# AlexGeControl/Visual-Inertial-Odometry

Measured on AMD Instinct MI355X. Metric: GN iterations/s, 11-frame (10-keyframe) window, 20k landmarks per GPU, higher is better.
Workload: dtype f64

## Files before the change

### visual-inertial-odometry_amd/csrc/vio_chain_core.h

```cpp
#ifndef VIO_CHAIN_CORE_H
#define VIO_CHAIN_CORE_H
#ifndef CH_DIAG_SKIP
#define CH_DIAG_SKIP 0
#endif

#ifdef VIO_STAMPS
#define CH_STAMP(slot) do { if (dbg && (tid & 63) == 0) { asm volatile("s_waitcnt lgkmcnt(0)" ::: "memory"); dbg[slot] = __builtin_amdgcn_s_memtime() - t_start__; } } while (0)
#else
#define CH_STAMP(slot) do { } while (0)
#endif

#ifdef VIO_STAMPS
__device__ unsigned long long *g_ch_dbg = nullptr;
__device__ unsigned long long g_ch_t0 = 0;
#define CH_TSTAMP(cond, slot) do { if ((cond) && g_ch_dbg && (threadIdx.x & 63) == 0) { g_ch_dbg[slot] = __builtin_amdgcn_s_memtime() - g_ch_t0; } } while (0)
#else
#define CH_TSTAMP(cond, slot) do { } while (0)
#endif
struct ChLane {
    int oA0, oA2;
    int oM0, oM2;
    int r16, g;
    bool r9;
};

__device__ __forceinline__ void ch_scan_tiles(double *P, int wi, int lane) {
    int *sNZ = (int *)(P + CH_OFF_NZ);
    for (int tile = wi; tile < 55; tile += 14) {
        const double *t = P + CH_OFF_SC + tile * CH_SCSZ;
        bool nz = t[lane] != 0.0 || t[lane + 64] != 0.0;
        if (lane + 128 < CH_SCSZ) nz = nz || t[lane + 128] != 0.0;
        const unsigned long long any = __ballot(nz);
        if (lane == 0) sNZ[tile] = any != 0ull ? 1 : 0;
    }
}
__device__ __forceinline__ unsigned long long ch_eff_mask(const double *P, int lane) {
    const int *sNZ = (const int *)(P + CH_OFF_NZ);
    const unsigned long long nz = __ballot(lane < 55 && sNZ[min(lane, 54)] != 0);
    unsigned long long eff = 0ull;
    unsigned a = 0, b = 0;
    for (int e = 0; e < 5; ++e) {
        a |= (unsigned)(nz >> (5 * e)) & 31u;
        b |= (unsigned)(nz >> (5 * (10 - e))) & 31u;
        eff |= (unsigned long long)a << (5 * e);
        eff |= (unsigned long long)b << (5 * (10 - e));
    }
    eff |= (unsigned long long)(((unsigned)(nz >> 25) & 31u) | a | b) << 25;
    return eff;
}
__device__ __forceinline__ bool ch_bit(unsigned long long eff, int e, int t) { return (eff >> (5 * e + t)) & 1ull; }

__device__ __forceinline__ void ch_chain_level(double *P, const ChLane &L, int e, int n, bool upd, int lane, double *scr) {
    double *sD = P + CH_OFF_D;
#ifdef VIO_STAMPS
    const unsigned long long ts0 = __builtin_amdgcn_s_memtime();
#endif
    if (e == 5) ch_factor<9, CH_TS, CH_TS>((lds_double *)(P + ch_sd(e)), (lds_double *)(P + CH_OFF_I9), (lds_double *)(P + ch_sm(e)), lane);
    else ch_factor<9, CH_TS, CH_TS, true>((lds_double *)(P + ch_sd(e)), (lds_double *)(P + CH_OFF_I9), (lds_double *)(P + ch_sm(e)), lane,
                                          (lds_double *)(P + ch_so(e)), (lds_double *)scr);
#ifdef VIO_STAMPS
    const unsigned long long ts1 = __builtin_amdgcn_s_memtime();
#endif
// ... 238 lines not shown
                ps_v4d acc2;
                ch_ld_c9(P + ch_sc(eB - 1, 0) + (wi - 5) * CH_SCSZ, L, acc2);
                ch_fused<eB, true>(P, L, wi - 5, acc2);
                ch_st_c9(P + ch_sc(eB - 1, 0) + (wi - 5) * CH_SCSZ, L, acc2);
            }
        }
        first_cc = wi >= 10 ? wi - 10 : wi + 3;
    } else {
        busy = wi < 5;
        if (wi < 5) {
            if (LEV == 4) {
                if (ch_bit(eff, 4, wi) || ch_bit(eff, 6, wi)) {
                    ps_v4d acc2;
                    ch_ld_c9(P + ch_sc(5, 0) + wi * CH_SCSZ, L, acc2);
                    if (ch_bit(eff, 4, wi)) ch_fused<4, true>(P, L, wi, acc2);
                    if (ch_bit(eff, 6, wi)) ch_fused<6, true>(P, L, wi, acc2);
                    ch_st_c9(P + ch_sc(5, 0) + wi * CH_SCSZ, L, acc2);
                }
            } else if (ch_bit(eff, 5, wi)) {
                ps_v4d dummy = {0.0, 0.0, 0.0, 0.0};
                ch_fused<5, false>(P, L, wi, dummy);
            }
        }
        first_cc = wi >= 5 ? wi - 5 : wi + 8;
    }
    if (CAM && LEV > 0 && wi < 5) {
        if (ch_bit(eff, LEV - 1, wi)) ch_yc_tile(P, LEV - 1, wi, lane);
        if (ch_bit(eff, 11 - LEV, wi)) ch_yc_tile(P, 11 - LEV, wi, lane);
    }
    if (CAM && LEV > 0) {
        if (LEV < 4) {
            if (wi >= 10 && wi < 13) { ch_cc_early(P, L, 2 * (wi - 10), LEV - 1, eff); ch_cc_early(P, L, 2 * (wi - 10) + 1, LEV - 1, eff); }
            else if (wi < 9) ch_cc_early(P, L, 6 + wi, LEV - 1, eff);
        } else if (wi < 5) {
            ch_cc_early(P, L, 10 + wi, LEV - 1, eff);
        } else if (wi < 13) {
            ch_cc_early(P, L, wi - 5, LEV - 1, eff);
            if (wi < 7) ch_cc_early(P, L, wi + 3, LEV - 1, eff);
        }
    }
    (void)first_cc;
    (void)busy;
}

__device__ __forceinline__ ChLane ch_lane(int lane) {
    const int r16 = lane & 15, g = lane >> 4;
    ChLane L;
    L.r16 = r16; L.g = g; L.r9 = r16 < 9;
    L.oA0 = r16 * CH_TS + g; L.oA2 = r16 * CH_TS + (g == 0 ? 8 : 9);
    L.oM0 = g * CH_TS + r16; L.oM2 = (g == 0) ? 8 * CH_TS + r16 : 8 * CH_TS + 9;
    return L;
}

template <bool CAM>
__device__ __forceinline__ unsigned long long ch_chain_elimination(double *P, const int tid, const ChLane &L, unsigned long long *dbg, unsigned long long t_start__,
                                                                   const bool scanned = false) {
    const int lane = tid & 63;
    const int uwave = __builtin_amdgcn_readfirstlane(tid >> 6);
    const int g = L.g;
    const bool r9 = L.r9;
    double *sD = P + CH_OFF_D;
    (void)dbg; (void)t_start__;
    unsigned long long eff = 0ull;
#ifndef CH_NO_PRIO
    if (uwave < 2) __builtin_amdgcn_s_setprio(3);
    else if (uwave == 15) __builtin_amdgcn_s_setprio(2);
#endif
    if (uwave < 2) {
        const int dir = uwave == 0 ? 1 : -1;
        int e = uwave == 0 ? 0 : 10;
        for (int lev = 0; lev < 6; ++lev, e += dir) {
            if (lev < 5 || uwave == 0) {
                if (lev == 5) {
                    double *td = P + ch_sd(5);
                    const double *so = P + ch_so(6);
                    const double a0 = so[L.oA0], a1 = so[L.oA0 + 4], a2 = so[L.oA2];
                    const double p0 = sD[6 * 16 + g], p1 = sD[6 * 16 + g + 4], p2 = sD[6 * 16 + g + 8];
                    ps_v4d acc = {td[L.oM0], td[L.oM0 + 4 * CH_TS], td[L.oM0 + 8 * CH_TS], 0.0};
                    acc = __builtin_amdgcn_mfma_f64_16x16x4f64(a0 * p0, -a0, acc, 0, 0, 0);
                    acc = __builtin_amdgcn_mfma_f64_16x16x4f64(a1 * p1, -a1, acc, 0, 0, 0);
                    acc = __builtin_amdgcn_mfma_f64_16x16x4f64(a2 * p2, -a2, acc, 0, 0, 0);
                    if (r9) { td[L.oM0] = acc[0]; td[L.oM0 + 4 * CH_TS] = acc[1]; if (g == 0) td[L.oM0 + 8 * CH_TS] = acc[2]; }
                }
                ch_chain_level(P, L, e, e + dir, !(uwave == 1 && lev == 4), lane, P + CH_OFF_X + 64 * uwave);
                if (uwave == 0) CH_STAMP(64 + 4 * lev);
            }
            CH_STAMP(256 + 16 * lev + uwave);
            __syncthreads();
            if (uwave == 0) CH_STAMP(65 + 4 * lev);
        }
        eff = ch_eff_mask(P, lane);
        if (uwave == 0) CH_STAMP(233);
        if (CAM) {
            if (uwave == 0) { if (ch_bit(eff, 5, 0)) { ps_v4d dummy = {0.0, 0.0, 0.0, 0.0}; ch_fused<5, false>(P, L, 0, dummy); } }
            else ch_cc_early(P, L, 0, 4, eff);
            if (uwave == 0) CH_STAMP(234);
            if (uwave == 1) CH_STAMP(235);
        }
        __syncthreads();
    } else {
        const int wi = uwave - 2;
        if (!scanned) ch_scan_tiles(P, wi, lane);
        CH_STAMP(256 + uwave);
        __syncthreads();
        eff = ch_eff_mask(P, lane);
        ch_worker_phase<0, CAM>(P, L, wi, lane, eff); if (uwave == 2) CH_STAMP(112);
        CH_STAMP(256 + 16 + uwave);
        __syncthreads();
        ch_worker_phase<1, CAM>(P, L, wi, lane, eff); if (uwave == 2) CH_STAMP(113);
        CH_STAMP(256 + 32 + uwave);
        __syncthreads();
        ch_worker_phase<2, CAM>(P, L, wi, lane, eff); if (uwave == 2) CH_STAMP(114); CH_STAMP(140 + uwave);
        CH_STAMP(256 + 48 + uwave);
        __syncthreads();
        ch_worker_phase<3, CAM>(P, L, wi, lane, eff); if (uwave == 2) CH_STAMP(115);
        CH_STAMP(256 + 64 + uwave);
        __syncthreads();
        ch_worker_phase<4, CAM>(P, L, wi, lane, eff); if (uwave == 2) CH_STAMP(116); CH_STAMP(180 + uwave);
        CH_STAMP(256 + 80 + uwave);
        __syncthreads();
        if (CAM) {
            if (wi >= 1 && wi < 5) { if (ch_bit(eff, 5, wi)) { ps_v4d dummy = {0.0, 0.0, 0.0, 0.0}; ch_fused<5, false>(P, L, wi, dummy); } }
            else if (wi == 13) ch_rhs_phase<5>(P, lane);
            else if (wi == 0 || (wi >= 5 && wi < 9)) {
                const int t = wi == 0 ? 0 : wi - 4;
                if (ch_bit(eff, 4, t)) ch_yc_tile(P, 4, t, lane);
                if (ch_bit(eff, 6, t)) ch_yc_tile(P, 6, t, lane);
            }
        } else {
            ch_worker_phase<5, CAM>(P, L, wi, lane, eff);
        }
        if (uwave == 2) CH_STAMP(117); CH_STAMP(200 + uwave);
        __syncthreads();
    }
    if (uwave == 0) CH_STAMP(87);
    return eff;
}

template <bool SPLIT, typename Mid1, typename Mid2>
__device__ __forceinline__ void ch_camera_solve(double *P, const int tid, const ChLane &L, const unsigned long long eff, Mid1 mid1, Mid2 mid2,
                                                unsigned long long *dbg, unsigned long long t_start__, const bool ext_trivial = false) {
    const int lane = tid & 63;
    const int uwave = __builtin_amdgcn_readfirstlane(tid >> 6);
    const int r16 = L.r16, g = L.g;
    const bool r9 = L.r9;
    double *sD = P + CH_OFF_D, *sX = P + CH_OFF_X, *sY = P + CH_OFF_Y, *sMc = P + CH_OFF_MC;
    (void)dbg; (void)t_start__;
    const int lofs = r16 * PS_TROW + g;
    const int cofs = g * PS_TROW + r16;
    if (SPLIT) {
#ifndef CH_NO_PRIO
        if (uwave == 0) __builtin_amdgcn_s_setprio(3);
        else if (uwave == 15) __builtin_amdgcn_s_setprio(2);
#endif
        if (uwave < 15) {
            int I, J;
            ch_tile_ij(uwave, I, J);
            double *tc = P + ch_cc(I, J) + cofs;
            ps_v4d acc;
#pragma unroll
            for (int v = 0; v < 4; ++v) acc[v] = tc[4 * PS_TROW * v];
            ch_cc_deferred_terms(P, L, I, J, acc, eff);
#pragma unroll
            for (int v = 0; v < 4; ++v) tc[4 * PS_TROW * v] = acc[v];
            if (uwave == 0) ch_factor_tile(P + ch_cc(0, 0), sMc, sD + CH_YC, 16, lane);
            else if (uwave >= 10) {
                const int t = uwave - 10;
#pragma unroll
                for (int i = 0; i < 11; ++i) {
                    const int e = (i == 10) ? 5 : ((i & 1) ? 10 - (i >> 1) : (i >> 1));
                    if (ch_bit(eff, e, t)) ch_yc_tile(P, e, t, lane);
                }
            }
        }
    } else
    if (uwave == 0) {
        double *tc = P + ch_cc(0, 0) + cofs;
        ps_v4d acc;
#pragma unroll
        for (int v = 0; v < 4; ++v) acc[v] = tc[4 * PS_TROW * v];
        if (ch_bit(eff, 5, 0)) ch_cc_term(P, L, 5, 0, 0, acc);
#pragma unroll
        for (int v = 0; v < 4; ++v) tc[4 * PS_TROW * v] = acc[v];
        ch_factor_tile(P + ch_cc(0, 0), sMc, sD + CH_YC, 16, lane);
    } else if (uwave == 15) {
        ch_yc_term<5>(P, lane);
    } else {
#ifndef CH_PREAMBLE_ALL_WAVES
        if ((uwave & 3) != 0) {
            ch_cc_last3(P, L, uwave, eff);
            if (uwave <= 3) ch_cc_last3(P, L, 4 * uwave, eff);
        }
#else
// ... 135 lines not shown
                if (g == 3) sX[CH_YC + 64 + r16] = x;
                __builtin_amdgcn_wave_barrier();
                asm volatile("" ::: "memory");
            }
            {
                const double *src = P + ch_cc(K, K) + r16 * PS_TROW;
#pragma unroll
                for (int j = 0; j < 16; ++j) mw[j] = src[j];
            }
#pragma unroll
            for (int J = 4; J >= 1; --J) {
                const double *src = P + ch_cc(J, min(K, J - 1)) + r16;
#pragma unroll
                for (int r = 0; r < 16; ++r) ucol[r] = src[r * PS_TROW];
                const double xj = sX[CH_YC + 16 * J + r16];
                PS_DOT16(acc, acc, xj, ucol);
                if (J >= 1) {
                    double x;
                    PS_DOT16(x, 0.0, own_v - acc, mw);
                    if (K == J - 1) sX[CH_YC + 16 * K + r16] = x;
                    __builtin_amdgcn_wave_barrier();
                    asm volatile("" ::: "memory");
                }
            }
        } else if (uwave < 11 && uwave != 5 && CH_DIAG_SKIP != 4) {
            const int e = uwave;
            const double *m = P + ch_sm(e) + k9 * CH_TS, *so = P + ch_so(e);
            double gk[3], mv[9], sv[3][9];
#pragma unroll
            for (int i = 0; i < 9; ++i) mv[i] = m[i];
#pragma unroll
            for (int v = 0; v < 3; ++v) {
                const int j = min(g + 4 * v, 8);
#pragma unroll
                for (int i = 0; i < 9; ++i) sv[v][i] = so[j * CH_TS + i];
            }
            __builtin_amdgcn_sched_barrier(0);
#pragma unroll
            for (int v = 0; v < 3; ++v) {
                double sum = 0.0;
#pragma unroll
                for (int i = 0; i < 9; ++i) sum = fma(mv[i], sv[v][i], sum);
                gk[v] = sum;
            }
            __builtin_amdgcn_sched_barrier(0);
            if (r9) {
                double *sg = P + ch_so(e) + k9 * CH_TS;
                sg[g] = gk[0]; sg[g + 4] = gk[1];
                if (g == 0) sg[8] = gk[2];
            }
        }
        if (uwave == 0) CH_STAMP(111);
        if (uwave == 15) CH_STAMP(170);
        __syncthreads();
        if ((uwave == 11 || uwave == 12) && CH_DIAG_SKIP != 4) {
            double gc[5][9], vc[5];
#pragma unroll
            for (int s2 = 0; s2 < 5; ++s2) {
                const int eb = (uwave == 11) ? 4 - s2 : 6 + s2;
                const double *src = P + ch_so(eb) + k9 * CH_TS;
#pragma unroll
                for (int j = 0; j < 9; ++j) gc[s2][j] = src[j];
            }
            __syncthreads();
            if (lane < 16) {
                double xs = sX[5 * 16 + k9];
#pragma unroll
                for (int s2 = 0; s2 < 5; ++s2) vc[s2] = sX[((uwave == 11) ? 4 - s2 : 6 + s2) * 16 + k9];
#pragma unroll
                for (int s2 = 0; s2 < 5; ++s2) {
                    const int eb = (uwave == 11) ? 4 - s2 : 6 + s2;
                    double t;
                    CH_DOT9(t, 0.0, xs, gc[s2]);
                    const double xn = vc[s2] - t;
                    if (r9) sX[eb * 16 + r16] = xn;
                    xs = xn;
                }
            }
            if (uwave == 11) CH_STAMP(175);
        } else {
            if (uwave == 13) {
                mid1(lane);
                CH_STAMP(171);
            } else if (uwave < 11 && CH_DIAG_SKIP != 4) {
                const int e = uwave;
                double sacc = 0.0, lv[5][4], xv[5][4];
#pragma unroll
                for (int t = 0; t < 5; ++t) {
                    if (ch_bit(eff, e, t)) {
                        const double *src = P + ch_sc(e, t) + g * CH_TS + k9;
                        const double *xj = sX + CH_YC + 16 * t + g;
#pragma unroll
                        for (int v = 0; v < 4; ++v) { lv[t][v] = src[4 * v * CH_TS]; xv[t][v] = xj[4 * v]; }
                    }
                }
                __builtin_amdgcn_sched_barrier(0);
#pragma unroll
                for (int t = 0; t < 5; ++t) {
                    if (ch_bit(eff, e, t)) {
#pragma unroll
                        for (int v = 0; v < 4; ++v) sacc = fma(lv[t][v], xv[t][v], sacc);
                    }
                }
                double *scr = P + CH_OFF_SD;
                scr[e * 64 + lane] = sacc;
                __builtin_amdgcn_wave_barrier();
                if (lane < 16) {
                    const double c = ((scr[e * 64 + r16] + scr[e * 64 + 16 + r16]) + scr[e * 64 + 32 + r16]) + scr[e * 64 + 48 + r16];
                    const double dd = sD[e * 16 + k9];
                    const double v = d_div(sY[e * 16 + k9], dd, d_fast_rcp(dd)) - c;
                    const double *src = P + ch_sm(e) + k9 * CH_TS;
                    double m9[9], gv;
#pragma unroll
                    for (int j = 0; j < 9; ++j) m9[j] = (j < k9) ? 0.0 : src[j];
                    CH_DOT9(gv, 0.0, v, m9);
                    if (r9) sX[e * 16 + r16] = gv;
                }
            }
            if (uwave == 0) CH_STAMP(172);
            __syncthreads();
            if (uwave == 0) CH_STAMP(173);
            mid2(uwave < 11 ? uwave : uwave - 2, lane);
            if (uwave == 0) CH_STAMP(174);
        }
        if (uwave == 0) CH_STAMP(63);
        d_lds_barrier();
    }
}

template <typename Mid1, typename Mid2>
__device__ __forceinline__ void ch_factor_solve(double *P, const int tid, Mid1 mid1, Mid2 mid2, unsigned long long *dbg = nullptr, const bool ext_trivial = false,
                                                const bool scanned = false) {
    unsigned long long t_start__ = 0ull;
#ifdef VIO_STAMPS
    t_start__ = __builtin_amdgcn_s_memtime();
    if (tid == 0) { g_ch_dbg = dbg; g_ch_t0 = t_start__; }
#endif
    const ChLane L = ch_lane(tid & 63);
    const unsigned long long eff = ch_chain_elimination<true>(P, tid, L, dbg, t_start__, scanned);
    ch_camera_solve<false>(P, tid, L, eff, mid1, mid2, dbg, t_start__, ext_trivial);
}
#endif
```

### visual-inertial-odometry_amd/csrc/vio_pose_solve_chain.h

```cpp
#ifndef VIO_POSE_SOLVE_CHAIN_H
#define VIO_POSE_SOLVE_CHAIN_H

#define CH_NS 11
#define CH_TS 11
#define CH_SCSZ (16 * CH_TS)
#define CH_S9SZ (9 * CH_TS)
#define CH_OFF_SC 0
#define CH_OFF_SO (CH_OFF_SC + CH_NS * 5 * CH_SCSZ)
#define CH_OFF_SD (CH_OFF_SO + 10 * CH_S9SZ)
#define CH_OFF_CC (CH_OFF_SD + CH_NS * CH_S9SZ)
#define CH_OFF_Y (CH_OFF_CC + 15 * PS_TS)
#define CH_YC 176
#define CH_NDIM 256
#define CH_PACKED ((CH_OFF_Y + CH_NDIM + 1) & ~1)
#define CH_SET_STRIDE 16128
#define CH_OFF_SM CH_PACKED
#define CH_OFF_MC (CH_OFF_SM + CH_NS * CH_S9SZ)
#define CH_OFF_D (CH_OFF_MC + PS_TS)
#define CH_OFF_X (CH_OFF_D + CH_NDIM)
#define CH_OFF_I9 (CH_OFF_X + CH_NDIM)
#define CH_OFF_I16 (CH_OFF_I9 + CH_S9SZ)
#define CH_OFF_NZ (CH_OFF_I16 + PS_TS)
#define CH_LDS_CORE (CH_OFF_NZ + 32)
static_assert(CH_NS * CH_S9SZ >= CH_NS * 64, "the back-substitution's scratch (11 x 64) lives in the SD tiles");
// ... 239 lines not shown
    if (t == i) {
        const double extra = d_rhs_rest(T, valid, i, cur);
        T.bs[i] = extra;
        T.bfull[wset * 176 + i] = extra;
        T.diagfull[i] = d_hs_rest(T, valid, i, i);
        T.Pg[wset * CH_SET_STRIDE + CH_OFF_Y + ch_dim(i)] = extra;
    }
}
__global__ __launch_bounds__(RED_THREADS) void k_reduce_c(ReduceTables R, DeviceTables T) { d_reduce_body<true>(R, &T); }
__global__ __launch_bounds__(RED_THREADS) void k_reduce_cb(BatchArgs a) {
    const DeviceTables T = d_batch_tables(a);
    const bool test_prev = (a.gn_flags & 1) != 0, err_prev = test_prev && T.has_prior;
    if ((int)blockIdx.x >= VIO_NPAIR + VIO_NCB + 1 + RED_SB_BLOCKS && !err_prev) return;
    const int loop = T.cur_hint == -2, cur = loop ? 0 : T.cur_hint;
    ReduceTables R{T.list_off, T.list, T.slab, T.vis, test_prev ? T.step_part : nullptr, T.n_items, a.gate, T.lm,
                   err_prev ? T.Jtinv : nullptr, err_prev ? T.bprior + cur * 176 : nullptr, err_prev ? T.errprior + cur * 160 : nullptr, loop};
    d_reduce_body<true>(R, &T);
}
__global__ __launch_bounds__(ASMC_THREADS) void k_assemble_cb(BatchArgs a) { const DeviceTables T = d_batch_tables(a); d_assemble_chain_body(T); }

#define CH_OFF_DX CH_LDS_CORE
#define CH_OFF_R (CH_OFF_DX + 176)
#define CH_OFF_B (CH_OFF_R + 112)
#define CH_OFF_STATE (CH_OFF_B + 176)
#define CH_LDS_DOUBLES (CH_OFF_STATE + 184)
template <bool SPLIT>
__device__ __forceinline__ void d_pose_solve_chain_body(const DeviceTables &T) {
    double *P = dyn_smem;
    double *sX = P + CH_OFF_X, *sDx = P + CH_OFF_DX, *sR = P + CH_OFF_R, *sB = P + CH_OFF_B, *sState = P + CH_OFF_STATE;
    const int tid = threadIdx.x;
    const int lane = tid & 63;
    const int uwave = __builtin_amdgcn_readfirstlane(tid >> 6);
    LmState *lm = T.lm;
    __shared__ LmRegs sLm;
    if (d_gated_off(lm, T.lm_gate)) return;
    const bool lm_loop = T.cur_hint == -2;
    int cur = lm_loop ? 0 : d_cur(T);
    double lambda = lm_loop ? 0.0 : lm->lambda;
    const int n = PS_N;
#ifdef VIO_STAMPS
    const unsigned long long t_start = __builtin_amdgcn_s_memtime();
#define CH_OUT(slot) do { if (tid == 0 && T.dbg) T.dbg[slot] = __builtin_amdgcn_s_memtime() - t_start; } while (0)
#else
#define CH_OUT(slot) do { } while (0)
#endif
    int set = lm_loop ? (lm->sys ^ lm->pending) : 0;
    const double *cfi = SPLIT ? T.cfi : nullptr;
    double xs0 = 0.0, xs1 = 0.0, xd = 0.0, xy = 0.0, xe = 0.0;
#ifndef CH_NO_EARLY_START
    const bool early = !SPLIT && !lm_loop && !(T.gn_flags & 32);
#else
    const bool early = false;
#endif
    const double bf_early = (early && tid >= 192 && tid < 192 + n) ? T.bfull[tid - 192] : 0.0;
    if (early) {
        const double *img = T.Pg;
        if (uwave < 2) {
            const int so0 = CH_OFF_SO + (uwave ? 5 * CH_S9SZ : 0), sd0 = CH_OFF_SD + (uwave ? 6 * CH_S9SZ : 0);
            const int nsd = uwave ? 5 * CH_S9SZ : 6 * CH_S9SZ, e0 = uwave ? 6 : 0, ne = uwave ? 5 : 6;
            double vo[8], vd[10];
#pragma unroll
            for (int q = 0; q < 8; ++q) vo[q] = img[so0 + min(lane + 64 * q, 5 * CH_S9SZ - 1)];
#pragma unroll
            for (int q = 0; q < 10; ++q) vd[q] = img[sd0 + min(lane + 64 * q, nsd - 1)];
            for (int i = lane; i < CH_S9SZ; i += 64) P[CH_OFF_I9 + i] = (i / CH_TS == i % CH_TS) ? 1.0 : 0.0;
            for (int i = lane; i < ne * CH_S9SZ; i += 64) P[CH_OFF_SM + e0 * CH_S9SZ + i] = 0.0;
            for (int i = lane; i < ne * 16; i += 64) P[CH_OFF_D + e0 * 16 + i] = 1.0;
#pragma unroll
            for (int q = 0; q < 8; ++q) P[so0 + min(lane + 64 * q, 5 * CH_S9SZ - 1)] = vo[q];
#pragma unroll
            for (int q = 0; q < 10; ++q) P[sd0 + min(lane + 64 * q, nsd - 1)] = vd[q];
            if (lane < ne * 9) P[ch_sd(e0 + lane / 9) + (lane % 9) * (CH_TS + 1)] += lambda;
        } else {
            const int wt = tid - 128;
            const double2 *src2 = reinterpret_cast<const double2 *>(img);
            double2 *dst2 = reinterpret_cast<double2 *>(P);
            double2 va[4], vb[4], vc[3];
            static_assert(CH_OFF_CC % 2 == 1 && CH_PACKED % 2 == 0 && (CH_PACKED - CH_OFF_CC - 1) / 2 <= 3 * 896, "the copy of the camera block below");
#pragma unroll
            for (int k = 0; k < 4; ++k) {
                const int t = min(uwave - 2 + 14 * k, 54);
                va[k] = src2[t * (CH_SCSZ / 2) + lane];
                vb[k] = src2[t * (CH_SCSZ / 2) + 64 + min(lane, CH_SCSZ / 2 - 65)];
            }
#pragma unroll
            for (int q = 0; q < 3; ++q) vc[q] = src2[min((CH_OFF_CC + 1) / 2 + wt + 896 * q, CH_PACKED / 2 - 1)];
            const double vc0 = img[CH_OFF_CC];
            double st[3] = {0.0, 0.0, 0.0}, er[3] = {0.0, 0.0, 0.0};
            const bool test_here = uwave == 2 && d_step_owed(T, 1);
            double tv[6] = {0.0, 0.0, 0.0, 0.0, 0.0, 0.0}, ichi = 0.0;
            if (test_here) {
                tv[0] = T.vis[VIS_CHI]; tv[1] = T.vis[VIS_STEP + 1]; tv[2] = lm->chi; tv[3] = T.sp_part[0]; tv[4] = T.sp_part[1]; tv[5] = T.sp_part[2];
                ichi = T.imu_out[min(lane, 9) * IMU_OUT + IMU_CHI];
            }
            if (uwave == 2) {
#pragma unroll
                for (int k = 0; k < 3; ++k) st[k] = T.state[cur * STATE_STRIDE + min(lane + 64 * k, STATE_STRIDE - 1)];
                if (test_here && T.has_prior) {
#pragma unroll
                    for (int k = 0; k < 3; ++k) if (lane + 64 * k < VIO_PRD) er[k] = T.errprior[cur * 160 + lane + 64 * k];
                }
            }
            for (int i = wt; i < PS_TS; i += 896) P[CH_OFF_I16 + i] = (i / PS_TROW == i % PS_TROW) ? 1.0 : 0.0;
            if (wt < CH_NDIM - CH_YC) P[CH_OFF_D + CH_YC + wt] = 1.0;
            int *sNZ = (int *)(P + CH_OFF_NZ);
#pragma unroll
            for (int k = 0; k < 4; ++k) {
                const int t = uwave - 2 + 14 * k;
                if (t < 55) {
                    dst2[t * (CH_SCSZ / 2) + lane] = va[k];
                    if (lane < CH_SCSZ / 2 - 64) dst2[t * (CH_SCSZ / 2) + 64 + lane] = vb[k];
                    const bool nz = va[k].x != 0.0 || va[k].y != 0.0 || (lane < CH_SCSZ / 2 - 64 && (vb[k].x != 0.0 || vb[k].y != 0.0));
                    const unsigned long long any = __ballot(nz);
                    if (lane == 0) sNZ[t] = any != 0ull ? 1 : 0;
                }
            }
            auto cam_value = [&](int o, double v) {
                if (o < CH_OFF_Y) {
                    const int ti = (o - CH_OFF_CC) / PS_TS, w = (o - CH_OFF_CC) % PS_TS, r = w / PS_TROW, c = w % PS_TROW;
                    const bool dtile = ti == 0 || ti == 2 || ti == 5 || ti == 9 || ti == 14;
                    if (dtile && r == c && c < 16) v = (ti == 14 && r >= 8) ? 1.0 : v + lambda;
                }
                return v;
            };
#pragma unroll
            for (int q = 0; q < 3; ++q) {
                const int i2 = (CH_OFF_CC + 1) / 2 + wt + 896 * q;
                if (i2 < CH_PACKED / 2) { double2 v = vc[q]; v.x = cam_value(2 * i2, v.x); v.y = cam_value(2 * i2 + 1, v.y); dst2[i2] = v; }
            }
            if (wt == 0) P[CH_OFF_CC] = cam_value(CH_OFF_CC, vc0);
            if (uwave == 2) {
#pragma unroll
                for (int k = 0; k < 3; ++k) if (lane + 64 * k < STATE_STRIDE) sState[lane + 64 * k] = st[k];
                if (test_here) {
                    double w[3];
#pragma unroll
                    for (int k = 0; k < 3; ++k) w[k] = d_wave_sum_to_lane63(er[k] * er[k]);
                    const int valid = d_imu_mask(T);
                    double t_imu = 0.0;
#pragma unroll
                    for (int k = 0; k < 10; ++k) { const double c = d_readlane(ichi, k); if ((valid >> k) & 1) t_imu += c; }
                    if (lane == 63) {
                        double total = tv[0] + t_imu;
                        if (T.has_prior) total += sqrt((w[0] + w[1]) + w[2]);
                        const double tempChi = 0.5 * total;
                        const double scale = 0.5 * (tv[1] + ((tv[3] + tv[4]) + tv[5])) + 1e-6;
                        lm->chi_try = tempChi;
                        lm->scale = scale;
                        lm->rho = (tv[2] - tempChi) / scale;
                        lm->trials += 1;
                        lm->chi = tempChi;
                        lm->cur = cur;
                        lm->accepted = 1;
                        lm->naccepted += 1;
                        lm->need_linearize = 1;
                        lm->false_cnt = 0;
                        if (!isfinite(tempChi)) lm->finite = 0;
                    }
                }
            }
        }
    } else {
    if (SPLIT) {
        xs0 = cfi[CH_OFF_SM + tid];
        if (tid < CH_NS * CH_S9SZ - PS_THREADS) xs1 = cfi[CH_OFF_SM + PS_THREADS + tid];
        if (tid < CH_YC) { xd = cfi[CH_OFF_D + tid]; xy = cfi[CH_OFF_Y + tid]; }
        if (tid < 2) xe = cfi[CH_OFF_NZ + tid];
    }
    for (int pass = 0; pass < 2; ++pass) {
        const double2 *src = reinterpret_cast<const double2 *>(T.Pg + set * CH_SET_STRIDE);
        const double2 *csrc = reinterpret_cast<const double2 *>(cfi);
        double2 *dst = reinterpret_cast<double2 *>(P);
        static_assert((CH_PACKED / 2 + PS_THREADS - 1) / PS_THREADS == 8, "copy below is written for 8 rounds");
        static_assert(CH_OFF_SD % 2 == 0, "the range that comes from cfi is whole double2s");
#define CH_FROM_CFI(i2) (SPLIT && (i2) < CH_OFF_SD / 2)
#define CH_LD(q) const double2 v##q = (CH_FROM_CFI(tid + q * PS_THREADS) ? csrc : src)[min(tid + q * PS_THREADS, CH_PACKED / 2 - 1)];
#define CH_ST(q) dst[min(tid + q * PS_THREADS, CH_PACKED / 2 - 1)] = v##q;
        CH_LD(0) CH_LD(1) CH_LD(2) CH_LD(3) CH_LD(4) CH_LD(5) CH_LD(6) CH_LD(7)
        if (pass == 0) {
            double stv = (tid < STATE_STRIDE) ? T.state[cur * STATE_STRIDE + tid] : 0.0;
            const double stv1 = (lm_loop && tid < STATE_STRIDE) ? T.state[STATE_STRIDE + tid] : 0.0;
            const bool test_here = d_step_owed(T, 1);
            double t_chi = 0.0, t_step = 0.0, t_lmchi = 0.0, t_imu = 0.0, t_sp = 0.0;
// ... 73 lines not shown
#undef CH_LD
#undef CH_ST
#undef CH_FROM_CFI
    }
    if (tid < n) {
        const int d = ch_dim(tid);
        if (d >= CH_YC) P[ch_cc_elem(d - CH_YC, d - CH_YC)] += lambda;
        else if (!SPLIT) P[ch_sd(d >> 4) + (d & 15) * (CH_TS + 1)] += lambda;
    } else if (tid < n + 8) {
        P[ch_cc_elem(72 + tid - n, 72 + tid - n)] = 1.0;
    } else if (tid >= 256 && tid < 256 + CH_S9SZ + PS_TS) {
        const int i = tid - 256;
        P[CH_OFF_I9 + i] = (i < CH_S9SZ) ? ((i / CH_TS == i % CH_TS) ? 1.0 : 0.0) : (((i - CH_S9SZ) / PS_TROW == (i - CH_S9SZ) % PS_TROW) ? 1.0 : 0.0);
    } else if (tid >= 640 && tid < 640 + CH_NDIM) {
        if (!SPLIT || tid - 640 >= CH_YC) P[CH_OFF_D + tid - 640] = 1.0;
    }
    if (SPLIT) {
        P[CH_OFF_SM + tid] = xs0;
        if (tid < CH_NS * CH_S9SZ - PS_THREADS) P[CH_OFF_SM + PS_THREADS + tid] = xs1;
        if (tid < CH_YC) { P[CH_OFF_D + tid] = xd; P[CH_OFF_Y + tid] = xy; }
        if (tid < 2) P[CH_OFF_NZ + tid] = xe;
    } else {
        for (int i = tid; i < CH_NS * CH_S9SZ; i += PS_THREADS) P[CH_OFF_SM + i] = 0.0;
    }
    __syncthreads();
    }
    CH_OUT(0);
    const int trial = cur ^ 1;
    const bool prior_here = T.has_prior && !(T.gn_flags & 4);
    const int lm_dim = T.lm_dim;
    double *pairtab_trial = T.pairtab + trial * PAIRTAB_STRIDE;
    double *pw = P + CH_OFF_CC;
    auto mid1 = [&](int ln) {
        if (prior_here || CH_DIAG_SKIP == 2) return;
        if (ln < 12) {
            const double *p = (ln == 0) ? sState + STATE_EXT : sState + STATE_POSE + 7 * (ln - 1);
            const double *d = (ln == 0) ? sX + CH_YC + 66 : sX + CH_YC + 6 * (ln - 1);
            double dd[6], tmp[7];
#pragma unroll
            for (int k = 0; k < 6; ++k) dd[k] = d[k];
            d_pose_plus(p, dd, tmp);
            double *q = (ln == 0) ? pw + STATE_EXT : pw + STATE_POSE + 7 * (ln - 1);
#pragma unroll
            for (int k = 0; k < 7; ++k) q[k] = tmp[k];
        }
        __builtin_amdgcn_wave_barrier();
        asm volatile("" ::: "memory");
        if (lm_dim != 3) d_pair_rotations(pw, pw + 96, ln);
    };
    auto mid2 = [&](int idx, int ln) {
        if (prior_here || lm_dim == 3 || CH_DIAG_SKIP == 1 || CH_DIAG_SKIP == 2) return;
        d_pair_rows(pw, pairtab_trial, pw + 96, ln + 64 * idx, 14 * 64);
    };
    const bool ext_trivial = T.ext_fixed && !T.marg_mode;
    if (SPLIT) {
        unsigned long long t0__ = 0ull;
#ifdef VIO_STAMPS
        t0__ = __builtin_amdgcn_s_memtime();
        if (tid == 0) { g_ch_dbg = T.dbg; g_ch_t0 = t0__; }
#endif
        const unsigned lo = (unsigned)P[CH_OFF_NZ], hi = (unsigned)P[CH_OFF_NZ + 1];
        const unsigned long long eff = ((unsigned long long)__builtin_amdgcn_readfirstlane(hi) << 32) | (unsigned long long)(unsigned)__builtin_amdgcn_readfirstlane(lo);
        ch_camera_solve<true>(P, tid, ch_lane(lane), eff, mid1, mid2, T.dbg, t0__, ext_trivial);
    } else {
        ch_factor_solve(P, tid, mid1, mid2, T.dbg, ext_trivial, early);
    }
    CH_OUT(2);
    for (int i = tid; i < n; i += PS_THREADS) sDx[i] = sX[ch_dim(i)];
    if (tid >= 192 && tid < 384 && T.sp_part) {
        const int i = tid - 192;
        const double dxi = (i < n) ? sX[ch_dim(min(i, n - 1))] : 0.0;
        const double bi = early ? bf_early : ((i < n) ? T.bfull[set * 176 + i] : 0.0);
        const double w = d_wave_sum_to_lane63((i < n) ? dxi * (lambda * dxi + bi) : 0.0);
        if (lane == 63) T.sp_part[i >> 6] = w;
    }
    if (!prior_here) {
        if (tid >= 128 && tid < 128 + 84) sState[tid - 128] = P[CH_OFF_CC + tid - 128];
        else if (tid >= 256 && tid < 256 + 99) { const int e = tid - 256; sState[STATE_SB + e] += sX[(e / 9) * 16 + (e % 9 < 3 ? 6 + e % 9 : (e % 9 < 6 ? e % 9 : e % 9 - 6))]; }
        d_lds_barrier();
        if (tid >= 192 && tid < 192 + n) T.dx[tid - 192] = sDx[tid - 192];
        if (tid >= 384 && tid < 384 + STATE_STRIDE) T.state[trial * STATE_STRIDE + (tid - 384)] = sState[tid - 384];
        CH_OUT(3);
        return;
    }
    __syncthreads();

    if (uwave < 2) {
        if (tid < 12) {
            double *p = (tid == 0) ? sState + STATE_EXT : sState + STATE_POSE + 7 * (tid - 1);
            const double *d = (tid == 0) ? sDx : sDx + 6 + 15 * (tid - 1);
            double tmp[7];
            d_pose_plus(p, d, tmp);
            for (int k = 0; k < 7; ++k) p[k] = tmp[k];
        } else if (tid >= 16 && tid < 16 + 99) {
            const int e = tid - 16, f = e / 9, k = e % 9;
            sState[STATE_SB + e] = sState[STATE_SB + e] + sDx[12 + 15 * f + k];
        }
        __syncthreads();
        if (T.lm_dim != 3) d_pair_rotations(sState, sR, tid);
        __syncthreads();
    } else {
        {
            double hp[PS_PRIOR_ROWS][3], bp[PS_PRIOR_ROWS];
#pragma unroll
            for (int r = 0; r < PS_PRIOR_ROWS; ++r) {
                const int i = (uwave - 2) + 14 * r;
#pragma unroll
                for (int q = 0; q < 3; ++q) {
                    const int j = lane + 64 * q;
                    hp[r][q] = (i < n && j < n) ? T.Hprior[i * n + j] : 0.0;
                }
                bp[r] = (i < n) ? T.bprior[cur * 176 + i] : 0.0;
            }
            const double x0 = sDx[lane], x1 = sDx[lane + 64], x2 = (lane + 128 < n) ? sDx[lane + 128] : 0.0;
#pragma unroll
            for (int r = 0; r < PS_PRIOR_ROWS; ++r) {
                const int i = (uwave - 2) + 14 * r;
                const double v = d_bprior_dot(hp[r][0], hp[r][1], hp[r][2], x0, x1, x2, bp[r]);
                if (lane == 63 && i < n) { sB[i] = v; T.bprior[trial * 176 + i] = v; }
            }
        }
        __syncthreads();
        double jp[PS_JT_ROWS][3];
#pragma unroll
        for (int r = 0; r < PS_JT_ROWS; ++r) {
            const int i = (uwave - 2) + 14 * r;
#pragma unroll
            for (int q = 0; q < 3; ++q) {
                const int j = lane + 64 * q;
                jp[r][q] = (i < VIO_PRD && j < VIO_PRD) ? T.Jtinv[i * VIO_PRD + j] : 0.0;
            }
        }
        __syncthreads();
        {
            const double y0 = sB[lane], y1 = sB[lane + 64], y2 = (lane + 128 < VIO_PRD) ? sB[lane + 128] : 0.0;
#pragma unroll
            for (int r = 0; r < PS_JT_ROWS; ++r) {
// ... 372 lines not shown
    if (tid == 0) sCnt[0] = 0;
    __syncthreads();
    if (tid == 0) for (int i = 1; i <= PS_THREADS; ++i) sCnt[i] += sCnt[i - 1];
    __syncthreads();
    int o = sCnt[tid];
    for (int q = 0; q < PER; ++q) {
        const int p = tid * PER + q;
        if (p < CH_OFF_CC) { const double v = T.prior_simg[p]; if (v != 0.0) { T.prior_list[128 + o] = p; T.prior_cval[o] = v; ++o; } }
    }
    if (tid == 0) {
        T.prior_list[0] = sCnt[PS_THREADS];
        int m = 0;
        for (int r = 0; r < 99; ++r) if (T.prior_flags[CPI_NTILES + r]) T.prior_list[2 + m++] = r;
        T.prior_list[1] = m;
    }
}

__global__ __launch_bounds__(PS_THREADS) void k_chain_pre(DeviceTables T) {
    double *P = dyn_smem;
    const int tid = threadIdx.x;
    const double lambda = T.lm->lambda;
    const double *img = T.Pg + d_set_w(T) * CH_SET_STRIDE;
    for (int i = tid; i < CH_OFF_CC; i += PS_THREADS) P[i] = img[i];
    if (tid < CH_YC) P[CH_OFF_Y + tid] = img[CH_OFF_Y + tid];
    ch_chain_pre_init(P, tid);
    __syncthreads();
    if (tid < CH_NS * 9) { const int e = tid / 9, k = tid % 9; P[ch_sd(e) + k * (CH_TS + 1)] += lambda; }
    __syncthreads();
    const unsigned long long eff = ch_chain_elimination<false>(P, tid, ch_lane(tid & 63), T.dbg, 0ull);
    ch_chain_pre_store(P, tid, eff, T.cfi);
}

#ifdef VIO_DEBUG_ENTRY_POINTS
__global__ __launch_bounds__(PS_THREADS) void k_chain_solve_test(const double *img, double lambda, double *x_nat, double *lds_dump) {
    double *P = dyn_smem;
    const int tid = threadIdx.x;
    for (int i = tid; i < CH_PACKED; i += PS_THREADS) P[i] = img[i];
    for (int i = CH_PACKED + tid; i < CH_LDS_CORE; i += PS_THREADS) P[i] = 0.0;
    __syncthreads();
    if (tid < PS_N) {
        const int d = ch_dim(tid);
        if (d >= CH_YC) P[ch_cc_elem(d - CH_YC, d - CH_YC)] += lambda;
        else P[ch_sd(d >> 4) + (d & 15) * (CH_TS + 1)] += lambda;
    } else if (tid < PS_N + 8) {
        P[ch_cc_elem(72 + tid - PS_N, 72 + tid - PS_N)] = 1.0;
    } else if (tid >= 256 && tid < 256 + CH_S9SZ + PS_TS) {
        const int i = tid - 256;
        P[CH_OFF_I9 + i] = (i < CH_S9SZ) ? ((i / CH_TS == i % CH_TS) ? 1.0 : 0.0) : (((i - CH_S9SZ) / PS_TROW == (i - CH_S9SZ) % PS_TROW) ? 1.0 : 0.0);
    } else if (tid >= 640 && tid < 640 + CH_NDIM) {
        P[CH_OFF_D + tid - 640] = 1.0;
    }
    for (int i = tid; i < CH_NS * CH_S9SZ; i += PS_THREADS) P[CH_OFF_SM + i] = 0.0;
    __syncthreads();
    ch_factor_solve(P, tid, [](int) {}, [](int, int) {});
    if (tid < PS_N) x_nat[tid] = P[CH_OFF_X + ch_dim(tid)];
    if (lds_dump) for (int i = tid; i < CH_LDS_CORE; i += PS_THREADS) lds_dump[i] = P[i];
}
#endif
#endif
#endif
```

Before: 20590.

## Defer camera-block LDS copy past phase 0 and issue pose/dx stores early

Splits the camera-block copy so the first two rounds are loaded into registers early but written to LDS only after worker phase 0, via a new 'late' callback hooked into the chain elimination. Also has an idle wave (uwave 14) write pose state and camera dx entries to global memory during the mid2 phase, and drops the trailing sState rewrite and barrier on the non-prior path. The aim is to overlap global loads and stores with the elimination work and shorten the serial tail after the solve. In exchange, register pressure rises from holding the deferred values across phase 0, and correctness depends on phase 0 not reading the deferred region, which a static_assert checks.

```diff
diff --git a/visual-inertial-odometry_amd/csrc/vio_chain_core.h b/visual-inertial-odometry_amd/csrc/vio_chain_core.h
--- a/visual-inertial-odometry_amd/csrc/vio_chain_core.h
+++ b/visual-inertial-odometry_amd/csrc/vio_chain_core.h
@@ -4,10 +4,20 @@
 #define CH_DIAG_SKIP 0
 #endif
 
+#ifndef CH_EARLY_POSE_STORES
+#define CH_EARLY_POSE_STORES 1
+#endif
+#ifndef CH_LATE_CAMERA_COPY
+#define CH_LATE_CAMERA_COPY 1
+#endif
+struct ChNoLate { __device__ __forceinline__ void operator()() const {} };
+
 #ifdef VIO_STAMPS
 #define CH_STAMP(slot) do { if (dbg && (tid & 63) == 0) { asm volatile("s_waitcnt lgkmcnt(0)" ::: "memory"); dbg[slot] = __builtin_amdgcn_s_memtime() - t_start__; } } while (0)
+#define CH_RSTAMP(cond, slot) do { if ((cond) && dbg && (tid & 63) == 0) { asm volatile("s_waitcnt lgkmcnt(0)" ::: "memory"); dbg[slot] = __builtin_amdgcn_s_memtime(); } } while (0)
 #else
 #define CH_STAMP(slot) do { } while (0)
+#define CH_RSTAMP(cond, slot) do { } while (0)
 #endif
 
 #ifdef VIO_STAMPS
@@ -352,9 +362,9 @@
     return L;
 }
 
-template <bool CAM>
+template <bool CAM, typename Late = ChNoLate>
 __device__ __forceinline__ unsigned long long ch_chain_elimination(double *P, const int tid, const ChLane &L, unsigned long long *dbg, unsigned long long t_start__,
-                                                                   const bool scanned = false) {
+                                                                   const bool scanned = false, Late late = Late()) {
     const int lane = tid & 63;
     const int uwave = __builtin_amdgcn_readfirstlane(tid >> 6);
     const int g = L.g;
@@ -386,6 +396,7 @@
                 if (uwave == 0) CH_STAMP(64 + 4 * lev);
             }
             CH_STAMP(256 + 16 * lev + uwave);
+            CH_RSTAMP(lev == 0, 240 + uwave);
             __syncthreads();
             if (uwave == 0) CH_STAMP(65 + 4 * lev);
         }
@@ -402,9 +413,12 @@
         const int wi = uwave - 2;
         if (!scanned) ch_scan_tiles(P, wi, lane);
         CH_STAMP(256 + uwave);
-        __syncthreads();
+        CH_RSTAMP(true, 240 + uwave);
+        __syncthreads();
+        CH_RSTAMP(uwave == 2, 232);
         eff = ch_eff_mask(P, lane);
         ch_worker_phase<0, CAM>(P, L, wi, lane, eff); if (uwave == 2) CH_STAMP(112);
+        late();
         CH_STAMP(256 + 16 + uwave);
         __syncthreads();
         ch_worker_phase<1, CAM>(P, L, wi, lane, eff); if (uwave == 2) CH_STAMP(113);
@@ -437,8 +451,8 @@
     return eff;
 }
 
-template <bool SPLIT, typename Mid1, typename Mid2>
-__device__ __forceinline__ void ch_camera_solve(double *P, const int tid, const ChLane &L, const unsigned long long eff, Mid1 mid1, Mid2 mid2,
+template <bool SPLIT, typename Mid1, typename Mid2, typename MidOut>
+__device__ __forceinline__ void ch_camera_solve(double *P, const int tid, const ChLane &L, const unsigned long long eff, Mid1 mid1, Mid2 mid2, MidOut mid_out,
                                                 unsigned long long *dbg, unsigned long long t_start__, const bool ext_trivial = false) {
     const int lane = tid & 63;
     const int uwave = __builtin_amdgcn_readfirstlane(tid >> 6);
@@ -680,6 +694,7 @@
         }
         if (uwave == 0) CH_STAMP(111);
         if (uwave == 15) CH_STAMP(170);
+        CH_RSTAMP(uwave == 15, 227);
         __syncthreads();
         if ((uwave == 11 || uwave == 12) && CH_DIAG_SKIP != 4) {
             double gc[5][9], vc[5];
@@ -706,10 +721,12 @@
                 }
             }
             if (uwave == 11) CH_STAMP(175);
+            CH_RSTAMP(true, 230 + uwave - 11);
         } else {
             if (uwave == 13) {
                 mid1(lane);
                 CH_STAMP(171);
+                CH_RSTAMP(true, 228);
             } else if (uwave < 11 && CH_DIAG_SKIP != 4) {
                 const int e = uwave;
                 double sacc = 0.0, lv[5][4], xv[5][4];
@@ -748,24 +765,29 @@
             if (uwave == 0) CH_STAMP(172);
             __syncthreads();
             if (uwave == 0) CH_STAMP(173);
+            CH_RSTAMP(uwave == 0, 229);
+            CH_RSTAMP(true, 352 + uwave);
+            if (CH_EARLY_POSE_STORES && uwave == 14) mid_out(lane);
             mid2(uwave < 11 ? uwave : uwave - 2, lane);
+            CH_RSTAMP(true, 368 + uwave);
             if (uwave == 0) CH_STAMP(174);
         }
         if (uwave == 0) CH_STAMP(63);
         d_lds_barrier();
-    }
-}
-
-template <typename Mid1, typename Mid2>
-__device__ __forceinline__ void ch_factor_solve(double *P, const int tid, Mid1 mid1, Mid2 mid2, unsigned long long *dbg = nullptr, const bool ext_trivial = false,
-                                                const bool scanned = false) {
+        CH_RSTAMP(uwave == 0, 236);
+    }
+}
+
+template <typename Mid1, typename Mid2, typename MidOut, typename Late = ChNoLate>
+__device__ __forceinline__ void ch_factor_solve(double *P, const int tid, Mid1 mid1, Mid2 mid2, MidOut mid_out, unsigned long long *dbg = nullptr, const bool ext_trivial = false,
+                                                const bool scanned = false, Late late = Late()) {
     unsigned long long t_start__ = 0ull;
 #ifdef VIO_STAMPS
     t_start__ = __builtin_amdgcn_s_memtime();
-    if (tid == 0) { g_ch_dbg = dbg; g_ch_t0 = t_start__; }
+    if (tid == 0) { g_ch_dbg = dbg; g_ch_t0 = t_start__; if (dbg) dbg[1] = t_start__; }
 #endif
     const ChLane L = ch_lane(tid & 63);
-    const unsigned long long eff = ch_chain_elimination<true>(P, tid, L, dbg, t_start__, scanned);
-    ch_camera_solve<false>(P, tid, L, eff, mid1, mid2, dbg, t_start__, ext_trivial);
-}
-#endif
+    const unsigned long long eff = ch_chain_elimination<true>(P, tid, L, dbg, t_start__, scanned, late);
+    ch_camera_solve<false>(P, tid, L, eff, mid1, mid2, mid_out, dbg, t_start__, ext_trivial);
+}
+#endif
diff --git a/visual-inertial-odometry_amd/csrc/vio_pose_solve_chain.h b/visual-inertial-odometry_amd/csrc/vio_pose_solve_chain.h
--- a/visual-inertial-odometry_amd/csrc/vio_pose_solve_chain.h
+++ b/visual-inertial-odometry_amd/csrc/vio_pose_solve_chain.h
@@ -315,6 +315,28 @@
 #else
     const bool early = false;
 #endif
+    auto cam_value = [&](int o, double v) {
+        if (o < CH_OFF_Y) {
+            const int ti = (o - CH_OFF_CC) / PS_TS, w = (o - CH_OFF_CC) % PS_TS, r = w / PS_TROW, c = w % PS_TROW;
+            const bool dtile = ti == 0 || ti == 2 || ti == 5 || ti == 9 || ti == 14;
+            if (dtile && r == c && c < 16) v = (ti == 14 && r >= 8) ? 1.0 : v + lambda;
+        }
+        return v;
+    };
+    double2 vc_late[2] = {make_double2(0.0, 0.0), make_double2(0.0, 0.0)};
+    double vc0_late = 0.0;
+    const bool late_cam = CH_LATE_CAMERA_COPY && early;
+    auto late_copy = [&]() {
+        if (!late_cam) return;
+        const int wt = tid - 128;
+        double2 *dst2 = reinterpret_cast<double2 *>(P);
+#pragma unroll
+        for (int q = 0; q < 2; ++q) {
+            const int i2 = (CH_OFF_CC + 1) / 2 + wt + 896 * q;
+            double2 v = vc_late[q]; v.x = cam_value(2 * i2, v.x); v.y = cam_value(2 * i2 + 1, v.y); dst2[i2] = v;
+        }
+        if (wt == 0) P[CH_OFF_CC] = cam_value(CH_OFF_CC, vc0_late);
+    };
     const double bf_early = (early && tid >= 192 && tid < 192 + n) ? T.bfull[tid - 192] : 0.0;
     if (early) {
         const double *img = T.Pg;
@@ -340,6 +362,7 @@
             double2 *dst2 = reinterpret_cast<double2 *>(P);
             double2 va[4], vb[4], vc[3];
             static_assert(CH_OFF_CC % 2 == 1 && CH_PACKED % 2 == 0 && (CH_PACKED - CH_OFF_CC - 1) / 2 <= 3 * 896, "the copy of the camera block below");
+            static_assert((CH_OFF_CC + 1) / 2 + 2 * 896 <= CH_OFF_Y / 2, "the right-hand side (read in phase 0) lies in the third round of that copy");
 #pragma unroll
             for (int k = 0; k < 4; ++k) {
                 const int t = min(uwave - 2 + 14 * k, 54);
@@ -347,8 +370,10 @@
                 vb[k] = src2[t * (CH_SCSZ / 2) + 64 + min(lane, CH_SCSZ / 2 - 65)];
             }
 #pragma unroll
-            for (int q = 0; q < 3; ++q) vc[q] = src2[min((CH_OFF_CC + 1) / 2 + wt + 896 * q, CH_PACKED / 2 - 1)];
+            for (int q = CH_LATE_CAMERA_COPY ? 2 : 0; q < 3; ++q) vc[q] = src2[min((CH_OFF_CC + 1) / 2 + wt + 896 * q, CH_PACKED / 2 - 1)];
+#if !CH_LATE_CAMERA_COPY
             const double vc0 = img[CH_OFF_CC];
+#endif
             double st[3] = {0.0, 0.0, 0.0}, er[3] = {0.0, 0.0, 0.0};
             const bool test_here = uwave == 2 && d_step_owed(T, 1);
             double tv[6] = {0.0, 0.0, 0.0, 0.0, 0.0, 0.0}, ichi = 0.0;
@@ -364,6 +389,13 @@
                     for (int k = 0; k < 3; ++k) if (lane + 64 * k < VIO_PRD) er[k] = T.errprior[cur * 160 + lane + 64 * k];
                 }
             }
+#if CH_LATE_CAMERA_COPY
+            __builtin_amdgcn_sched_barrier(0);
+#pragma unroll
+            for (int q = 0; q < 2; ++q) vc_late[q] = src2[(CH_OFF_CC + 1) / 2 + wt + 896 * q];
+            vc0_late = img[CH_OFF_CC];
+            __builtin_amdgcn_sched_barrier(0);
+#endif
             for (int i = wt; i < PS_TS; i += 896) P[CH_OFF_I16 + i] = (i / PS_TROW == i % PS_TROW) ? 1.0 : 0.0;
             if (wt < CH_NDIM - CH_YC) P[CH_OFF_D + CH_YC + wt] = 1.0;
             int *sNZ = (int *)(P + CH_OFF_NZ);
@@ -378,20 +410,14 @@
                     if (lane == 0) sNZ[t] = any != 0ull ? 1 : 0;
                 }
             }
-            auto cam_value = [&](int o, double v) {
-                if (o < CH_OFF_Y) {
-                    const int ti = (o - CH_OFF_CC) / PS_TS, w = (o - CH_OFF_CC) % PS_TS, r = w / PS_TROW, c = w % PS_TROW;
-                    const bool dtile = ti == 0 || ti == 2 || ti == 5 || ti == 9 || ti == 14;
-                    if (dtile && r == c && c < 16) v = (ti == 14 && r >= 8) ? 1.0 : v + lambda;
-                }
-                return v;
-            };
-#pragma unroll
-            for (int q = 0; q < 3; ++q) {
+#pragma unroll
+            for (int q = CH_LATE_CAMERA_COPY ? 2 : 0; q < 3; ++q) {
                 const int i2 = (CH_OFF_CC + 1) / 2 + wt + 896 * q;
                 if (i2 < CH_PACKED / 2) { double2 v = vc[q]; v.x = cam_value(2 * i2, v.x); v.y = cam_value(2 * i2 + 1, v.y); dst2[i2] = v; }
             }
+#if !CH_LATE_CAMERA_COPY
             if (wt == 0) P[CH_OFF_CC] = cam_value(CH_OFF_CC, vc0);
+#endif
             if (uwave == 2) {
 #pragma unroll
                 for (int k = 0; k < 3; ++k) if (lane + 64 * k < STATE_STRIDE) sState[lane + 64 * k] = st[k];
@@ -571,20 +597,31 @@
         if (prior_here || lm_dim == 3 || CH_DIAG_SKIP == 1 || CH_DIAG_SKIP == 2) return;
         d_pair_rows(pw, pairtab_trial, pw + 96, ln + 64 * idx, 14 * 64);
     };
+    auto mid_out = [&](int ln) {
+        if (prior_here) return;
+        T.state[trial * STATE_STRIDE + ln] = pw[ln];
+        if (ln < STATE_SB - 64) T.state[trial * STATE_STRIDE + 64 + ln] = pw[64 + ln];
+        const int c0 = cam_to_full(ln);
+        T.dx[c0] = sX[ch_dim(c0)];
+        if (ln < 72 - 64) { const int c1 = cam_to_full(64 + ln); T.dx[c1] = sX[ch_dim(c1)]; }
+    };
     const bool ext_trivial = T.ext_fixed && !T.marg_mode;
     if (SPLIT) {
         unsigned long long t0__ = 0ull;
 #ifdef VIO_STAMPS
         t0__ = __builtin_amdgcn_s_memtime();
-        if (tid == 0) { g_ch_dbg = T.dbg; g_ch_t0 = t0__; }
+        if (tid == 0) { g_ch_dbg = T.dbg; g_ch_t0 = t0__; if (T.dbg) T.dbg[1] = t0__; }
 #endif
         const unsigned lo = (unsigned)P[CH_OFF_NZ], hi = (unsigned)P[CH_OFF_NZ + 1];
         const unsigned long long eff = ((unsigned long long)__builtin_amdgcn_readfirstlane(hi) << 32) | (unsigned long long)(unsigned)__builtin_amdgcn_readfirstlane(lo);
-        ch_camera_solve<true>(P, tid, ch_lane(lane), eff, mid1, mid2, T.dbg, t0__, ext_trivial);
+        ch_camera_solve<true>(P, tid, ch_lane(lane), eff, mid1, mid2, mid_out, T.dbg, t0__, ext_trivial);
     } else {
-        ch_factor_solve(P, tid, mid1, mid2, T.dbg, ext_trivial, early);
+        ch_factor_solve(P, tid, mid1, mid2, mid_out, T.dbg, ext_trivial, early, late_copy);
     }
     CH_OUT(2);
+#if CH_EARLY_POSE_STORES
+    if (prior_here)
+#endif
     for (int i = tid; i < n; i += PS_THREADS) sDx[i] = sX[ch_dim(i)];
     if (tid >= 192 && tid < 384 && T.sp_part) {
         const int i = tid - 192;
@@ -593,6 +630,19 @@
         const double w = d_wave_sum_to_lane63((i < n) ? dxi * (lambda * dxi + bi) : 0.0);
         if (lane == 63) T.sp_part[i >> 6] = w;
     }
+#if CH_EARLY_POSE_STORES
+    if (!prior_here) {
+        if (tid >= 512 && tid < 512 + n) { const int i = tid - 512, d = ch_dim(i); if (d < CH_YC) T.dx[i] = sX[d]; }
+        else if (tid >= 768 && tid < 768 + STATE_STRIDE - STATE_SB) {
+            const int e = tid - 768;
+            double v = sState[STATE_SB + e];
+            if (e < 99) v += sX[(e / 9) * 16 + (e % 9 < 3 ? 6 + e % 9 : (e % 9 < 6 ? e % 9 : e % 9 - 6))];
+            T.state[trial * STATE_STRIDE + STATE_SB + e] = v;
+        }
+        CH_OUT(3);
+        return;
+    }
+#else
     if (!prior_here) {
         if (tid >= 128 && tid < 128 + 84) sState[tid - 128] = P[CH_OFF_CC + tid - 128];
         else if (tid >= 256 && tid < 256 + 99) { const int e = tid - 256; sState[STATE_SB + e] += sX[(e / 9) * 16 + (e % 9 < 3 ? 6 + e % 9 : (e % 9 < 6 ? e % 9 : e % 9 - 6))]; }
@@ -602,6 +652,7 @@
         CH_OUT(3);
         return;
     }
+#endif
     __syncthreads();
 
     if (uwave < 2) {
@@ -1080,7 +1131,7 @@
     }
     for (int i = tid; i < CH_NS * CH_S9SZ; i += PS_THREADS) P[CH_OFF_SM + i] = 0.0;
     __syncthreads();
-    ch_factor_solve(P, tid, [](int) {}, [](int, int) {});
+    ch_factor_solve(P, tid, [](int) {}, [](int, int) {}, [](int) {});
     if (tid < PS_N) x_nat[tid] = P[CH_OFF_X + ch_dim(tid)];
     if (lds_dump) for (int i = tid; i < CH_LDS_CORE; i += PS_THREADS) lds_dump[i] = P[i];
 }
```

Result: no change. 20640 (median of 2 runs) (+0.3%).
